# ALIZE-Speaker-Recognition/LIA_RAL

Measured on AMD Instinct MI355X. Metric: Gframe-Gaussian evals/s (UBM EM pass: LLK + full-posterior statistics), higher is better.
Workload: dtype f64; 1 GPU; TrainWorld EM: 2048-Gaussian diag UBM, 60-dim float32 frames, 10000000 frames per GPU resident in HBM, 1 EM iteration per step; gaussians=2048, dim=60, frames_per_gpu=10000000, partitioning=frames sharded per rank, one RCCL all-reduce of 247810 doubles per step

## Files before the change

lia_ral_amd/csrc/capi_gmm.hip:

```cpp
#include <math.h>
#include <stdarg.h>
#include <stdlib.h>

#include "ctx.h"
#include "gmm_kernels.h"
#include "tv_kernels.h"
#include "capi_gmm_util.h"

static thread_local char g_err[512] = "";

static thread_local gmmiv_kopts g_kopts_val;
static thread_local const gmmiv_kopts *g_kopts_src = nullptr;
const gmmiv_kopts &gmmiv_kopts_cur() { return g_kopts_val; }
void gmmiv_kopts_bind(const gmmiv_kopts *ko) { g_kopts_val = ko ? *ko : gmmiv_kopts(); g_kopts_src = ko; }

void gmmiv_set_error(const char *fmt, ...)
{
    va_list ap;
    va_start(ap, fmt);
    vsnprintf(g_err, sizeof(g_err), fmt, ap);
    va_end(ap);
}

bool gmmiv_is_device_ptr(const void *p)
// ... 55 lines not shown
        GCHK(krc);
    }
    return GMMIV_OK;
}

int run_lse(gmmiv_ctx *c, const gmmiv_gmm *g, const XView &xv, int dt, int64_t T, double **lse_out)
{
    void *lse;
    int rc = c->scratch(WS_LSE, (size_t)(T > 0 ? T : 1) * sizeof(double), &lse);
    if (rc) return rc;
    if (g->KS == GMMK_KS_GENERIC) {
        if ((rc = topc_big(c, g, xv, dt, T, 1, 1, -INFINITY, INFINITY, nullptr, nullptr, nullptr, nullptr, nullptr, (double *)lse))) return rc;
        GCHK(count_dead(c, (const double *)lse, T));
        *lse_out = (double *)lse;
        return GMMIV_OK;
    }
    c->t_begin("k_llk_mfma");
    GCHK(gmmk_llk(c->stream, g->KS, dt == GMMIV_F64, xv.d, T, xv.ldx, g->D, g->Pt, g->nct, (double *)lse, (int)(c->use_glds | (c->dbg << 8)), (int)c->wg_waves));
    c->t_end();
    GCHK(count_dead(c, (const double *)lse, T));
    *lse_out = (double *)lse;
    return GMMIV_OK;
}

static int64_t z_chunk_frames(gmmiv_ctx *c, const gmmiv_gmm *g)
{
    if (!c->stats_z || g->KS > 15 || c->wg_waves != 8) return 0;
    int64_t tc = gmmiv_z_budget_frames(c, g->nct, 16);
    const int64_t round = (int64_t)c->n_cu * 2 * 256;
    tc = tc >= round ? tc / round * round : tc / 64 * 64;
    return tc >= 4096 ? tc : 0;
}

static int llk_z_run(gmmiv_ctx *c, const gmmiv_gmm *g, const XView &xv, int dt, int64_t c0, int64_t n, double *lse, const gmmk_zview &z, bool first)
{
    c->t_begin("k_llk_mfma", first);
    GCHK(gmmk_llk_z(c->stream, g->KS, dt == GMMIV_F64, gmmiv_x_at(xv, dt, c0), n, xv.ldx, g->D, g->Pt, g->nct, lse,
                    (int)(c->use_glds | ((c->dbg & 15) << 8)), z));
    c->t_end();
    return GMMIV_OK;
}

int generic_gamma_gemm(gmmiv_ctx *c, const gmmiv_gmm *g, const XView &xv, int dt, int64_t t0, int64_t n, const double *lse, bool sq, int NC,
                       double *S)
{
    int rc;
    int64_t per = (int64_t)(((size_t)512 << 20) / ((size_t)g->C * sizeof(double)));
    if (per < 64) per = 64;
    per = per / 2 * 2;
    void *gam, *xa;
    const int64_t first = n < per ? n : per;
    if ((rc = c->scratch(WS_Z, (size_t)(first > 0 ? first : 1) * g->C * sizeof(double), &gam))) return rc;
    if ((rc = c->scratch(WS_INV, (size_t)(first > 0 ? first : 1) * NC * sizeof(double), &xa))) return rc;
    if (n <= 0) { GCHK(hipMemsetAsync(S, 0, (size_t)g->C * NC * sizeof(double), c->stream)); return GMMIV_OK; }
    for (int64_t b = 0; b < n; b += per) {
        const int64_t m = n - b < per ? n - b : per;
        c->t_begin("k_posteriors", b == 0);
        GCHK(gmmk_posteriors(c->stream, dt == GMMIV_F64, gmmiv_x_at(xv, dt, t0 + b), (long)m, xv.ldx, g->D, g->C, g->Cp64, g->meanT, g->ivT, g->lwc, lse + t0 + b,
                             (double *)gam));
        c->t_end();
        GCHK(gmmk_build_xa(c->stream, dt == GMMIV_F64, gmmiv_x_at(xv, dt, t0 + b), xv.ldx, g->D, (long)m, sq ? 1 : 0, NC, (double *)xa));
        GCHK(tvk_dgemm(c->stream, true, false, g->C, NC, (int)m, 1.0, (const double *)gam, g->C, 0, (const double *)xa, NC, 0, b == 0 ? 0.0 : 1.0, S, NC, 0, 1));
    }
    return GMMIV_OK;
}

extern "C" {

const char *gmmiv_last_error(void) { return g_err; }
const char *gmmiv_version(void) { return "gmmiv 0.1 (gfx950)"; }

int gmmiv_ctx_create(int device, void *stream, gmmiv_ctx **out)
{
    if (!out) { gmmiv_set_error("ctx_create: out == NULL"); return GMMIV_ERR_ARG; }
    int ndev = 0;
    hipError_t e = hipGetDeviceCount(&ndev);
    if (e != hipSuccess || ndev <= 0) {
        (void)hipGetLastError();
        gmmiv_set_error("ctx_create: no HIP device available (%s)", e == hipSuccess ? "count = 0" : hipGetErrorString(e));
        return GMMIV_ERR_HIP;
    }
    if (device < 0 || device >= ndev) { gmmiv_set_error("ctx_create: device %d out of range [0,%d)", device, ndev); return GMMIV_ERR_ARG; }
    GCHK(hipSetDevice(device));
    gmmiv_ctx *c = new gmmiv_ctx();
    c->device = device;
    if (stream == GMMIV_STREAM_DEFAULT || stream == (void *)hipStreamLegacy) { c->stream = nullptr; c->own_stream = false; }
    else if (stream) { c->stream = (hipStream_t)stream; c->own_stream = false; }
    else { GCHK(hipStreamCreateWithFlags(&c->stream, hipStreamNonBlocking)); c->own_stream = true; }
    hipDeviceProp_t prop;
    if (hipGetDeviceProperties(&prop, device) == hipSuccess) { c->n_cu = prop.multiProcessorCount; c->total_mem = prop.totalGlobalMem; }
    if (hipMalloc((void **)&c->d_zero_llk, 2 * sizeof(unsigned long long)) != hipSuccess || hipMemset(c->d_zero_llk, 0, 2 * sizeof(unsigned long long)) != hipSuccess) {
        (void)hipGetLastError();
        if (c->own_stream) (void)hipStreamDestroy(c->stream);
        delete c;
        gmmiv_set_error("ctx_create: hipMalloc of the context's device counters failed");
        return GMMIV_ERR_HIP;
    }
    c->d_screened = c->d_zero_llk + 1;
    *out = c;
    return GMMIV_OK;
}

void gmmiv_ctx_destroy(gmmiv_ctx *c)
{
    if (!c) return;
    (void)hipSetDevice(c->device);
    (void)hipStreamSynchronize(c->stream);
    for (gmmiv_comm *cm : std::vector<gmmiv_comm *>(c->comms)) gmmiv_comm_orphan(cm);
    for (int i = 0; i < WS_COUNT; ++i)
        if (c->ws[i]) (void)hipFree(c->ws[i]);
    for (int i = 0; i < gmmiv_ctx::NSLOT; ++i) {
        for (hipEvent_t e : c->ev0[i]) (void)hipEventDestroy(e);
        for (hipEvent_t e : c->ev1[i]) (void)hipEventDestroy(e);
    }
    if (c->d_zero_llk) (void)hipFree(c->d_zero_llk);
    if (c->own_stream) (void)hipStreamDestroy(c->stream);
    if (g_kopts_src == &c->ko) gmmiv_kopts_bind(nullptr);
    delete c;
}

int gmmiv_ctx_sync(gmmiv_ctx *c)
{
    if (!c) return GMMIV_ERR_ARG;
    GCHK(hipStreamSynchronize(c->stream));
    return GMMIV_OK;
}

void *gmmiv_ctx_stream(gmmiv_ctx *c) { return c ? (void *)c->stream : nullptr; }

long gmmiv_ctx_set_option(gmmiv_ctx *c, const char *key, long value)
{
    if (!c || !key) return -1;
    long *slot = nullptr;
    if (!strcmp(key, "glds")) slot = &c->use_glds;
    else if (!strcmp(key, "em_chunks")) slot = &c->em_chunks;
    else if (!strcmp(key, "timing")) slot = &c->timing;
    else if (!strcmp(key, "wg_waves")) slot = &c->wg_waves;
    else if (!strcmp(key, "dbg")) slot = &c->dbg;
    else if (!strcmp(key, "prune_log2")) slot = &c->prune_log2;
    else if (!strcmp(key, "stats_z")) slot = &c->stats_z;
    else if (!strcmp(key, "z_scratch_mb")) slot = &c->z_scratch_mb;
    else if (!strcmp(key, "models_scratch_mb")) slot = &c->models_scratch_mb;
    else if (!strcmp(key, "trials_scratch_mb")) slot = &c->trials_scratch_mb;
    else if (!strcmp(key, "trials_piece")) slot = &c->trials_piece;
    else if (!strcmp(key, "tv_batch")) slot = &c->tv_batch;
    else if (!strcmp(key, "tv_tett_direct")) slot = &c->tv_tett_direct;
    else if (!strcmp(key, "tv_stats_split")) slot = &c->tv_stats_split;
    else if (!strcmp(key, "topc_z")) slot = &c->topc_z;
// ... 598 lines not shown
    if (rc) return rc;
    GCHK(gmmk_fill_chunks(c->stream, (long *)buf, nseg, (long)per, (long)T));
    *dev = (long *)buf;
    return GMMIV_OK;
}

static int em_stats_z(gmmiv_ctx *c, const gmmiv_gmm *g, const XView &xv, int dt, int64_t T, int64_t Tc, double weight,
                      double *lse, int *nseg_out, void **part_out)
{
    int rc;
    const int ngrp = gmmk_stats_z_groups(g->nct);
    int nseg = c->em_chunks > 0 ? (int)c->em_chunks : (c->n_cu * gmmk_stats_z_wg_per_cu() + ngrp - 1) / ngrp;
    nseg = (nseg + 7) / 8 * 8;
    const int64_t first = T < Tc ? T : Tc;
    const int64_t cap = (first + 255) / 256;
    if (nseg > cap) nseg = (int)((cap + 7) / 8 * 8);
    const int64_t nchunk = (T + Tc - 1) / Tc;
    const int64_t lastn = T - (nchunk - 1) * Tc;
    void *seg, *part;
    if ((rc = c->scratch(WS_SEG, 2 * (size_t)(nseg + 1) * sizeof(long), &seg))) return rc;
    auto fill = [&](long *dst, int64_t n) {
        const int64_t per = ((n + nseg - 1) / nseg + 63) / 64 * 64;
        return gmmk_fill_chunks(c->stream, dst, nseg, (long)per, (long)n);
    };
    GCHK(fill((long *)seg, first));
    GCHK(fill((long *)seg + nseg + 1, lastn));
    gmmk_zview z;
    if ((rc = gmmiv_z_reserve(c, g->nct, first, !(c->dbg & 64), &z, nullptr))) return rc;
    const int RL = gmmk_rl_for_ks(g->KS);
    const size_t Cp = (size_t)g->nct * 16;
    if ((rc = c->scratch(WS_PART, (size_t)nseg * Cp * 2 * RL * sizeof(double), &part))) return rc;
    for (int64_t k = 0; k < nchunk; ++k) {
        const int64_t c0 = k * Tc, n = (k == nchunk - 1) ? lastn : Tc;
        if ((rc = llk_z_run(c, g, xv, dt, c0, n, lse + c0, z, k == 0))) return rc;
        GCHK(count_dead(c, lse + c0, n));
        c->t_begin("k_stats_z", k == 0);
        GCHK(gmmk_stats_z(c->stream, g->KS, 1, dt == GMMIV_F64, gmmiv_x_at(xv, dt, c0), xv.ldx, g->D, g->C, g->nct, z, weight,
                          (const long *)seg + (k == nchunk - 1 ? nseg + 1 : 0), nseg, (double *)part, nullptr, 0, k > 0, c->prune_thr()));
        c->t_end();
    }
    *nseg_out = nseg;
    *part_out = part;
    return GMMIV_OK;
}

int gmmiv_em_accumulate(gmmiv_ctx *c, const gmmiv_gmm *g, const void *x, int dt, int64_t T, int64_t ldx, double weight,
                        double *acc)
{
    int rc = check_model(c, g);
    if (rc) return rc;
    if (T < 0 || !acc || !(weight > 0.0)) { gmmiv_set_error("em_accumulate: bad argument (T >= 0, weight > 0, acc != NULL)"); return GMMIV_ERR_ARG; }
    const size_t nacc = gmmiv_em_acc_len(g->C, g->D);
    DevOut<double> o;
    if ((rc = o.init(c, WS_T0, acc, nacc, true))) return rc;
    if (T == 0) return o.finish();
    XView xv;
    if ((rc = xv.init(c, x, dt, T, ldx, g->D))) return rc;
    if ((rc = count_unusable(c, xv, dt, T, g->D))) return rc;
    const int64_t Tc = z_chunk_frames(c, g);
    if (Tc > 0) {
        void *lsew, *small, *part;
        int nseg = 0;
        if ((rc = c->scratch(WS_LSE, (size_t)T * sizeof(double), &lsew))) return rc;
        if ((rc = c->scratch(WS_SMALL, 3 * 256 * sizeof(double), &small))) return rc;
        if ((rc = em_stats_z(c, g, xv, dt, T, Tc, weight, (double *)lsew, &nseg, &part))) return rc;
        GCHK(gmmk_llk_finalize(c->stream, (const double *)lsew, T, -INFINITY, INFINITY, nullptr, (double *)small, 0.0, weight, nullptr,
                               o.d + nacc - 2, weight, o.d + nacc - 1));
        GCHK(gmmk_em_reduce(c->stream, (const double *)part, nseg, g->C, g->nct * 16, g->D, g->KS, o.d));
        return o.finish();
    }
    double *lse;
    if ((rc = run_lse(c, g, xv, dt, T, &lse))) return rc;
    void *small;
    if ((rc = c->scratch(WS_SMALL, 3 * 256 * sizeof(double), &small))) return rc;
    GCHK(gmmk_llk_finalize(c->stream, lse, T, -INFINITY, INFINITY, nullptr, (double *)small, 0.0, weight, nullptr,
                           o.d + nacc - 2, weight, o.d + nacc - 1));
    if (g->KS == GMMK_KS_GENERIC) {
        const int NC = 2 * g->D + 2;
        void *S;
        if ((rc = c->scratch(WS_PART, (size_t)g->C * NC * sizeof(double), &S))) return rc;
        if ((rc = generic_gamma_gemm(c, g, xv, dt, 0, T, lse, true, NC, (double *)S))) return rc;
        GCHK(gmmk_scatter_em(c->stream, g->C, g->D, NC, (const double *)S, weight, o.d));
        return o.finish();
    }
    const int nw = c->wg_waves == 8 ? 8 : 4;
    const int ngrp = (g->nct + nw - 1) / nw;
    int nseg = c->em_chunks > 0 ? (int)c->em_chunks : ((nw == 8 ? 2 : 4) * c->n_cu + ngrp - 1) / ngrp;
    nseg = (nseg + 7) / 8 * 8;
    const int64_t cap = (T + 4095) / 4096;
    if (nseg > cap) nseg = (int)cap;
    if (nseg < 1) nseg = 1;
    long *seg;
// ... 519 lines not shown
```

lia_ral_amd/csrc/ctx.h:

```cpp
#pragma once
#include <hip/hip_runtime.h>
#include <stdint.h>
#include <stdio.h>
#include <string.h>
#include <stdlib.h>
#include <time.h>

#include <map>
#include <string>
#include <vector>

#include "../../include/gmmiv.h"

void gmmiv_set_error(const char *fmt, ...);

#include "kopts.h"

#define GBIND(c)                                                                                    \
    do {                                                                                            \
        GCHK(hipSetDevice((c)->device));                                                            \
        gmmiv_kopts_bind(&(c)->ko);                                                                 \
    } while (0)

#define GCHK(expr)                                                                                  \
// ... 4 lines not shown
            return GMMIV_ERR_HIP;                                                                   \
        }                                                                                           \
    } while (0)

enum { WS_X = 0, WS_LSE, WS_PART, WS_SEG, WS_SMALL, WS_T0, WS_T1, WS_T2, WS_T3, WS_T4, WS_T5, WS_T6, WS_T7, WS_T8,
       WS_T9, WS_TIV, WS_LP, WS_AUX, WS_SLAB, WS_SLOTS, WS_FLAGS, WS_Z, WS_EIT, WS_INV,
       WS_GFLAG, WS_NORM, WS_FEAT_OFF, WS_FEAT_OUT, WS_FEAT_IDX, WS_FEAT_M0, WS_FEAT_M1, WS_FEAT_M2, WS_FEAT_M3,
       WS_NORM_OFF, WS_NORM_STATE, WS_NORM_DECAY,
       WS_MB_PT, WS_MB_TILES, WS_MB_IDS, WS_MB_SEG, WS_MB_OFF, WS_MB_FTILES, WS_MB_OFFSRC,
       WS_TR_IDX, WS_TR_NLLK, WS_TR_LLKW, WS_TR_TILES, WS_TR_TAB, WS_TR_PART, WS_TR_ROW,
       WS_COUNT };

struct gmmiv_ctx {
    int device = 0;
    hipStream_t stream = nullptr;
    bool own_stream = false;
    void *ws[WS_COUNT] = {};
    size_t ws_size[WS_COUNT] = {};
    long use_glds = 1;
    long em_chunks = 0;
    long timing = 0;
    long dbg = 0;
    long prune_log2 = 0;
    double prune_arg() const { return prune_log2 > 0 ? -(double)prune_log2 * 0.6931471805599453 : -__builtin_inf(); }
    double prune_thr() const { return prune_log2 > 0 ? __builtin_ldexp(1.0, -(int)prune_log2) : 0.0; }
    long wg_waves = 8;
    long stats_z = 1;
    long topc_use_lanes = 4;
    long topc_rank2 = 1;
    long topc_rank_direct = 0;
    long topc_fused = 1;
    long assume_finite = 0;
    unsigned long long *d_zero_llk = nullptr, *d_screened = nullptr;
    long topc_fallbacks = 0;
    long topc_z = 1;
    long tv_acc_mb = 8192;
    long tv_md_device = 1;
    long tv_mstep_solve = 1;
    long tv_stats_split = 1;
    long tv_tett_direct = 1;
    long tv_batch = 1024;
    gmmiv_kopts ko;
    struct Hook { gmmiv_hook_fn fn = nullptr; void *user = nullptr; void call() const { if (fn) fn(user); } };
    Hook hook_tv_a_ready, hook_md_factored;
    long z_scratch_mb = 16384;
    long models_scratch_mb = 2048;
    long trials_scratch_mb = 2048;
    long trials_piece = 0;
    int n_cu = 256;
    std::vector<double> plda_ftjf;
    struct PldaK { std::vector<double> K; double alpha; };
    std::map<long, PldaK> plda_k;
    std::vector<struct gmmiv_comm *> comms;
    size_t total_mem = 0;
    enum { NSLOT = 6 };
    std::vector<hipEvent_t> ev0[NSLOT], ev1[NSLOT];
    const char *ev_name[NSLOT] = {};
    int ev_used[NSLOT] = {};
    int ev_cur = -1, ev_last = -1;

    int scratch(int slot, size_t bytes, void **out)
    {
        if (bytes == 0) bytes = 8;
        if (ws_size[slot] < bytes) {
            if (ws[slot]) {
                GCHK(hipStreamSynchronize(stream));
// ... 133 lines not shown
```

lia_ral_amd/csrc/devutil.h:

```cpp
#pragma once
#include <hip/hip_runtime.h>
#include <stdint.h>

typedef double d4 __attribute__((ext_vector_type(4)));

#define MFMA_F64(a, b, c) __builtin_amdgcn_mfma_f64_16x16x4f64((a), (b), (c), 0, 0, 0)

#define GMMIV_NEG_BIG (-1.0e300)
#define GMMIV_ZERO_LLK (-745.1332191019412)
#define GMMIV_PAD_LOGIT (-1.0e9)

__device__ __forceinline__ double gexp(double x)
{
    x = fmax(x, -750.0);
    const double n = __builtin_rint(x * 1.4426950408889634074);
    double r = __builtin_fma(n, -6.93147180369123816490e-01, x);
    r = __builtin_fma(n, -1.90821492927058770002e-10, r);
    double p = 1.6059043836821613e-10;
    p = __builtin_fma(p, r, 2.08767569878681e-09);
    p = __builtin_fma(p, r, 2.505210838544172e-08);
    p = __builtin_fma(p, r, 2.755731922398589e-07);
    p = __builtin_fma(p, r, 2.7557319223985893e-06);
    p = __builtin_fma(p, r, 2.48015873015873e-05);
    p = __builtin_fma(p, r, 1.984126984126984e-04);
// ... 37 lines not shown
    double r = __builtin_fma(k, -0.021660849219188094, x);
    r = __builtin_fma(k, -1.733101967801894e-10, r);
    const int ki = (int)k;
    const double tj = tab[ki & 31];
    double p = 1.984126984126984e-04;
    p = __builtin_fma(p, r, 1.388888888888889e-03);
    p = __builtin_fma(p, r, 8.333333333333333e-03);
    p = __builtin_fma(p, r, 4.1666666666666664e-02);
    p = __builtin_fma(p, r, 1.6666666666666666e-01);
    p = __builtin_fma(p, r, 0.5);
    p = __builtin_fma(p, r, 1.0);
    p = p * r;
    int n = (ki >> 5) - E;
    n = n < -2000 ? -2000 : n;
    return __builtin_ldexp(__builtin_fma(tj, p, tj), n);
}
#ifndef GEXP_TAB_BITS
#define GEXP_TAB_BITS 11
#endif
#define GEXP_TAB_N (1 << GEXP_TAB_BITS)
#if GEXP_TAB_BITS == 11
#define GEXP_TAB_SCALE 2954.639443740597
#define GEXP_TAB_HI 0.00033845076904981397
#define GEXP_TAB_LO 2.7079718246904592e-12
#define GEXP_TAB_LN2N 0.00033845077175778578
#elif GEXP_TAB_BITS == 6
#define GEXP_TAB_SCALE 92.33248261689366
#define GEXP_TAB_HI 0.010830424609594047
#define GEXP_TAB_LO 8.66550983900947e-11
#define GEXP_TAB_LN2N 0.010830424696249145
#else
#error "GEXP_TAB_BITS must be 6 or 11"
#endif
__device__ __forceinline__ void gexp_tab_init(double *tab, int tid, int nthreads)
{
    for (int j = tid; j < GEXP_TAB_N; j += nthreads) tab[j] = exp2((double)j * (1.0 / GEXP_TAB_N));
}
__device__ __forceinline__ double gexp_tab_poly(double r)
{
#if GEXP_TAB_BITS == 11
    double p = 1.6666666666666666e-01;
#else
    double p = 8.333333333333333e-03;
    p = __builtin_fma(p, r, 4.1666666666666664e-02);
    p = __builtin_fma(p, r, 1.6666666666666666e-01);
#endif
    p = __builtin_fma(p, r, 0.5);
    p = __builtin_fma(p, r, 1.0);
    return p * r;
}
__device__ __forceinline__ void gexp_tab_reduce(double x, int &ki, double &r)
{
    const double k = __builtin_rint(x * GEXP_TAB_SCALE);
#ifdef GEXP_TAB_TWO_STEP
    r = __builtin_fma(k, -GEXP_TAB_HI, x);
    r = __builtin_fma(k, -GEXP_TAB_LO, r);
#else
    r = __builtin_fma(k, -GEXP_TAB_LN2N, x);
#endif
    ki = (int)k;
}
__device__ __forceinline__ double gexp_tab_finish(int ki, double r, int E, const double *tab)
{
    const double tj = tab[ki & (GEXP_TAB_N - 1)];
    return __builtin_ldexp(__builtin_fma(tj, gexp_tab_poly(r), tj), (ki >> GEXP_TAB_BITS) - E);
}
__device__ __forceinline__ double gexp_tab_scaled(double x, int E, const double *tab)
{
    int ki;
// ... 154 lines not shown
```

lia_ral_amd/csrc/gmm_kernels.h:

```cpp
#pragma once
#include <hip/hip_runtime.h>

#include "kopts.h"
#include "../../include/gmmiv.h"

#define GMMK_KS_GENERIC 99
#define GMMK_MAX_DIM 4096
int gmmk_ks_for_dim(int D);
int gmmk_rl_for_ks(int KS);
int gmmk_pack_model(hipStream_t st, int C, int D, int KS, int nct, int Cp64, const double *w, const double *mean,
                    const double *iv, double *a, double *lwc, double *Pt, double *meanT, double *ivT);
int gmmk_llk(hipStream_t st, int KS, int x_f64, const void *x, long T, long ldx, int D, const double *Pt, int nct,
             double *lse, int use_glds, int wg_waves);
int gmmk_llk_finalize(hipStream_t st, const double *lse, long T, double lo, double hi, double *llk_out,
                      double *partial , double scale_c, double scale_r, double *dst_clamped,
                      double *dst_raw, double scale_n = 0.0, double *dst_count = nullptr);
int gmmk_add_scalar(hipStream_t st, double *dst, double v);
int gmmk_count_dead(hipStream_t st, const double *lse, long T, unsigned long long *cnt);
int gmmk_rows_sum_groups(hipStream_t st, long n, int ngroups, const int *rb, const double *src, double *dst);
int gmmk_stats(hipStream_t st, int KS, int sq, int x_f64, const void *x, long ldx, int D, int C, const double *Pt,
               int nct, const double *lse, double lse_shift, const long *seg_begin, int nseg, double *out0,
               double *out1, int mode, int wg_waves, double prune_arg);
int gmmk_em_reduce(hipStream_t st, const double *part, int nseg, int C, int Cp, int D, int KS, double *acc);
int gmmk_em_get(hipStream_t st, int C, int D, const double *acc, const double *prev_mean, const double *prev_cov,
// ... 10 lines not shown
int gmmk_topc_determine_big(hipStream_t st, int x_f64, const void *x, long T, long ldx, int D, int C, int Cp,
                            const double *meanT, const double *ivT, const double *lwc, const double *w, int ctop,
                            int complete, double lo, double hi, int *idx, double *lk, double *nlk, double *nllk,
                            double *nw, double *llk, double *zs);
int gmmk_topc_use_big(hipStream_t st, int x_f64, const void *x, long T, long ldx, int D, const double *mean,
                      const double *iv, const double *lwc, int C, int ctop, const int *idx, const double *nllk, int complete,
                      double lo, double hi, double *llk);
int gmmk_topc_use(hipStream_t st, int x_f64, const void *x, long T, long ldx, int D, const double *mean,
                  const double *iv, const double *lwc, int C, int ctop, const int *idx, const double *nllk, int complete,
                  double lo, double hi, double *llk);
int gmmk_frame_moments(hipStream_t st, int x_f64, const void *x, long T, long ldx, int D, double *partial,
                       int max_blocks, double *acc);
int gmmk_variance_control(hipStream_t st, int C, int D, double *cov, double flooring, double ceiling,
                          const double *cov_signal, unsigned long long *counts);
int gmmk_reciprocal(hipStream_t st, long n, const double *in, double *out);
int gmmk_gather_frames(hipStream_t st, int x_f64, const void *x, long ldx, int D, const long *idx, long n, void *out);
int gmmk_segment_means(hipStream_t st, const double *v, long ld, const long *item, long nitem, double *part, const long *pair_off,
                       const long *pair_len, long npair, double *out);
int gmmk_topgauss_select(hipStream_t st, long T, int cap, double mass, int fixed_count, const double *w, int *idx, const double *lk,
                         const double *llk, int *count, double *snsw, double *snsl, unsigned long long *capped);
int gmmk_flag_frames(hipStream_t st, int x_f64, const void *x, long T, long ldx, int D, unsigned char *flag, int *any);
int gmmk_fill_chunks(hipStream_t st, long *dst, int nseg, long per, long n);
int gmmk_count_flags(hipStream_t st, const unsigned char *flag, long T, unsigned long long *cnt);
int gmmk_gather_runs(hipStream_t st, int x_f64, const void *x, long ldx, int D, const long *runs, long nrun, void *out);

struct gmmk_zview {
    double *zbuf;
    long nfb;
    int *eit;
    double *inv;
    int *efin;
};
int gmmk_llk_z(hipStream_t st, int KS, int x_f64, const void *x, long T, long ldx, int D, const double *Pt, int nct,
               double *lse, int use_glds, const gmmk_zview &z);
int gmmk_llk_models(hipStream_t st, int KS, int x_f64, const void *x, long ldx, int D, const double *Pt, long pt_stride, int nct,
                    const gmmiv_model_tile *tiles, long ntiles, double *lse, int use_glds);
int gmmk_llk_z_models(hipStream_t st, int KS, int x_f64, const void *x, long ldx, int D, const double *Pt, long pt_stride, int nct,
                      const gmmiv_model_tile *tiles, long ntiles, double *lse, int use_glds, const gmmk_zview &z);
int gmmk_const_models(hipStream_t st, int G, int C, int Cp, int D, const double *w, long sw, const double *mean, long sm, const double *iv,
                      long si, double *a, double *lwc);
int gmmk_pack_models(hipStream_t st, int n, const int *ids, int C, int Cp, int D, int KS, int nct, const double *mean, long sm,
                     const double *iv, long si, const double *a, double *Pt);
int gmmk_llk_seg_finalize(hipStream_t st, const double *lse, const long *sb, long nseg, double lo, double hi, double *llk_out, double *seg_sum,
                          double *seg_llk);
int gmmk_map_adapt_models(hipStream_t st, int G, int C, int D, const double *N, const double *F, const double *count, long count_stride,
                          const double *w0, const double *mean0, const double *cur, long cur_stride, int method, int mean_adapt,
                          int weight_adapt, double mean_reg, double weight_reg, double mean_alpha, double *mean_out, double *w_out);
int gmmk_map_adapt_models_full(hipStream_t st, int G, int C, int D, const double *N, const double *F, const double *S, const double *count,
                               long count_stride, const double *w0, const double *mean0, const double *cov0, const double *cur_mean,
                               long cur_mean_stride, const double *cur_cov, long cur_cov_stride, int method, int mean_adapt, int var_adapt,
                               int weight_adapt, double mean_reg, double var_reg, double weight_reg, double mean_alpha, double *mean_out,
                               double *cov_out, double *w_out, int *status);
int gmmk_normalize_models(hipStream_t st, int G, int C, int D, const double *w, long w_stride, double *mean, double *cov, int nb_it,
                          int mean_only);
int gmmk_acc_to_rows(hipStream_t st, int C, int D, const double *acc, double *Nrow, double *Frow, double *Srow);
int gmmk_topc_cap(void);
int gmmk_llk_topc(hipStream_t st, int KS, int x_f64, const void *x, long T, long ldx, int D, const double *Pt, int nct, int use_glds,
                  int ctop, double *cand, int *cnt, double *theta, double *slow, int *efin);
int gmmk_topc_rank(hipStream_t st, int x_f64, const void *x, long n, long ldx, int D, int C, const double *cand, const int *cnt,
                   const double *theta, const double *slow, const int *efin, const double *mean, const double *iv, const double *lwc,
                   const double *w, int ctop, int complete, double lo, double hi, int *idx, double *lk, double *nlk, double *nllk,
                   double *nw, double *llk, int *flag, long *redo, int stats, long *wide);
int gmmk_topc_scatter(hipStream_t st, long n, int ctop, const long *redo, const int *sidx, const double *slk, const double *snlk,
                      const double *snllk, const double *snw, const double *sllk, int *idx, double *lk, double *nlk, double *nllk, double *nw,
                      double *llk);
int gmmk_posteriors(hipStream_t st, int x_f64, const void *x, long T, long ldx, int D, int C, int Cp, const double *meanT,
                    const double *ivT, const double *lwc, const double *lse, double *gamma);
// ... 40 lines not shown
```

lia_ral_amd/csrc/gmm_kernels.hip:

```cpp
#include <atomic>
#include "devutil.h"
#include "lds_attr.h"
#include "gmm_kernels.h"

typedef double d2v __attribute__((ext_vector_type(2)));

__device__ __forceinline__ void gmm_const_one(int c, int C, int D, const double *__restrict__ w, const double *__restrict__ mean,
                                              const double *__restrict__ iv, double *__restrict__ a, double *__restrict__ logwcst)
{
    if (c >= C) { a[c] = GMMIV_NEG_BIG; logwcst[c] = GMMIV_NEG_BIG; return; }
    double sl = 0.0, sm = 0.0;
    for (int d = 0; d < D; ++d) {
        double v = iv[(size_t)c * D + d], m = mean[(size_t)c * D + d];
        sl += log(v);
        sm += m * m * v;
    }
    double lw = (w[c] > 0.0) ? log(w[c]) : GMMIV_NEG_BIG;
    double lc = lw - 0.5 * D * 1.8378770664093454836 + 0.5 * sl;
    lc = fmax(lc, GMMIV_NEG_BIG);
    logwcst[c] = lc;
    a[c] = fmax(lc - 0.5 * sm, GMMIV_NEG_BIG);
}
__global__ void k_gmm_const(int C, int Cp, int D, const double *__restrict__ w,
                            const double *__restrict__ mean, const double *__restrict__ iv,
// ... 44 lines not shown
    long total = (long)nct * (2 * KS + 2) * 64;
    if (e >= total) return;
    Pt[e] = gmm_pack_one(e, C, D, KS, mean, iv, a);
}
__global__ void k_gmm_pack_batch(int C, int Cp, int D, int KS, int nct, const int *__restrict__ ids, const double *__restrict__ mean, long sm,
                                 const double *__restrict__ iv, long si, const double *__restrict__ a, double *__restrict__ Pt)
{
    long e = (long)blockIdx.x * blockDim.x + threadIdx.x;
    long total = (long)nct * (2 * KS + 2) * 64;
    if (e >= total) return;
    const size_t g = (size_t)ids[blockIdx.y];
    Pt[(size_t)blockIdx.y * total + e] = gmm_pack_one(e, C, D, KS, mean + g * sm, iv + g * si, a + g * Cp);
}

__global__ void k_gmm_transpose(int C, int Cp, int D, const double *__restrict__ mean,
                                const double *__restrict__ iv, double *__restrict__ meanT,
                                double *__restrict__ ivT)
{
    long e = (long)blockIdx.x * blockDim.x + threadIdx.x;
    if (e >= (long)D * Cp) return;
    int c = e % Cp, d = e / Cp;
    meanT[e] = c < C ? mean[(size_t)c * D + d] : 0.0;
    ivT[e] = c < C ? iv[(size_t)c * D + d] : 0.0;
}

#define TOPC_CAP 256
#define GMMIV_MIN_FRAME_EXP (-1076)
#ifndef K1_ABL
#define K1_ABL 0
#endif
#ifndef K1_PLAIN_SHARED
#define K1_PLAIN_SHARED 1
#endif
template <int KS, typename XT, int NW, int MODE, bool MM = false>
__global__ __launch_bounds__(NW * 64, 2) void k_llk_mfma(const void *__restrict__ x, long T, long ldx, int D,
                                                  const double *__restrict__ Pt, int nct,
                                                  double *__restrict__ lse_out, int use_glds, int dbg,
                                                  double *__restrict__ zbuf, long nfb, int *__restrict__ eit,
                                                  double *__restrict__ inv_out, int *__restrict__ efin_out,
                                                  const gmmiv_model_tile *__restrict__ tiles, long pt_stride)
{
    constexpr bool WZ = MODE == 1, TC = MODE == 2;
    static_assert(!MM || (MODE != 2 && NW == 8), "a model per segment: plain and stored-likelihood modes, 8 waves");
    constexpr int NR = 2 * KS + 2;
    constexpr int GT = 2;
    constexpr int TILE_D = GT * NR * 64;
    constexpr int PIECES = TILE_D * 8 / 1024;
    extern __shared__ __attribute__((aligned(16))) char smem[];
    double *buf0 = (double *)smem;
    double *buf1 = buf0 + TILE_D;
    double *etab = buf1 + TILE_D;
    int *ccnt = (int *)(etab + GEXP_TAB_N);

    const int tid = threadIdx.x, lane = tid & 63, wave = tid >> 6;
    const int i16 = lane & 15, q = lane >> 4;
    long tb0 = (long)blockIdx.x * (NW * 32);
    long wlo = 0, whi = 0, olo = 0, ohi = 0;
    if constexpr (MM) {
        const gmmiv_model_tile me = tiles[blockIdx.x];
        tb0 = me.first; wlo = me.lo; whi = me.hi; olo = me.lo - me.pad_lo; ohi = me.hi + me.pad_hi;
        Pt += (size_t)me.model * pt_stride;
    }
    const long tb = tb0 + wave * 32;
    gexp_tab_init(etab, tid, NW * 64);
    if (TC) ccnt[tid >> 1] = 0;

    constexpr int NA = TC ? KS : 2 * KS;
    double A[2][NA];
#pragma unroll
    for (int h = 0; h < 2; ++h) {
        const long t = tb + h * 16 + i16;
#pragma unroll
        for (int s = 0; s < KS; ++s) {
            const int k = 4 * s + q;
            double v = 0.0;
            if ((MM ? (t >= wlo && t < whi) : t < T) && k < D) v = feat_load<XT>::get(x, t * ldx + k);
            A[h][s] = v;
            if (!TC) A[h][NA - KS + s] = v * v;
        }
    }

    const int ntiles = nct / GT;
    auto stage = [&](double *dst, int tile) {
        const char *src = (const char *)(Pt + (size_t)tile * TILE_D);
        if (use_glds) {
            if (PIECES % NW == 0) {
#pragma unroll
                for (int j = 0; j < PIECES / NW; ++j) {
                    const int p = wave + NW * j;
                    __builtin_amdgcn_global_load_lds(
                        (const __attribute__((address_space(1))) void *)(src + p * 1024 + lane * 16),
                        (__attribute__((address_space(3))) void *)((char *)dst + p * 1024), 16, 0, 0);
                }
            } else {
                for (int p = wave; p < PIECES; p += NW)
                    __builtin_amdgcn_global_load_lds(
                        (const __attribute__((address_space(1))) void *)(src + p * 1024 + lane * 16),
                        (__attribute__((address_space(3))) void *)((char *)dst + p * 1024), 16, 0, 0);
            }
        } else {
            for (int p = wave; p < PIECES; p += NW) {
                uint4 v = *(const uint4 *)(src + p * 1024 + lane * 16);
                *(uint4 *)((char *)dst + p * 1024 + lane * 16) = v;
            }
        }
    };

    double sacc[2][4];
    int E[2][4], nref[2][4];
#pragma unroll
    for (int h = 0; h < 2; ++h)
#pragma unroll
// ... 263 lines not shown
                    if (need & (1u << (h * 4 + r)))
                        sacc[h][r] += gexp_tab_scaled(acc[0][h][r], E[h][r], etab) + gexp_tab_scaled(acc[1][h][r], E[h][r], etab);
        }
    };
    stage(buf0, 0);
    __syncthreads();
    auto step = [&](int tl, bool staged, bool is_late, bool first) __attribute__((always_inline)) {
        double *cur = (tl & 1) ? buf1 : buf0;
        double *nxt = (tl & 1) ? buf0 : buf1;
        if (staged && (TC || dbg < 2) && !(K1_ABL & 16)) stage(nxt, tl + 1);
        if (!is_late) {
            mfma_phase(cur);
            epi_phase(tl);
        } else {
            if (!first) epi_phase(tl - 1);
            mfma_phase(cur);
        }
        if (WZ) {
            if (is_late) asm volatile("s_waitcnt vmcnt(0)" ::: "memory");
            if (!(K1_ABL & 16)) asm volatile("s_waitcnt lgkmcnt(0)\n\ts_barrier" ::: "memory");
        } else {
            __syncthreads();
        }
    };
    if (!late) {
        for (int tl = 0; tl + 1 < ntiles; ++tl) step(tl, true, false, false);
        if (ntiles > 0) step(ntiles - 1, false, false, false);
    } else {
        if (ntiles > 1) step(0, true, true, true);
        for (int tl = 1; tl + 1 < ntiles; ++tl) step(tl, true, true, false);
        if (ntiles > 0) step(ntiles - 1, false, true, ntiles == 1);
    }
    if (late && ntiles > 0) epi_phase(ntiles - 1);
#pragma unroll
    for (int h = 0; h < 2; ++h)
#pragma unroll
        for (int r = 0; r < 4; ++r) {
            int Em = E[h][r];
#pragma unroll
            for (int o = 1; o < 16; o <<= 1) { const int oe = __shfl_xor(Em, o, 64); Em = oe > Em ? oe : Em; }
            int sh = E[h][r] - Em;
            sh = sh < -2000 ? -2000 : sh;
            double sv = __builtin_ldexp(sacc[h][r], sh);
#pragma unroll
            for (int o = 1; o < 16; o <<= 1) sv += shfl_xor_f64(sv, o);
            const long t = tb + h * 16 + q + 4 * r;
            if (TC) {
                if (i16 == 0 && t < T) { lse_out[t] = (double)thf[h][r]; inv_out[t] = sv; efin_out[t] = Em; }
                continue;
            }
            if (i16 == 0 && (MM ? (t >= wlo && t < whi) : t < T)) {
                const bool ok = sv > 0.0 && sv < __builtin_inf() && Em > GMMIV_MIN_FRAME_EXP;
                lse_out[t] = ok ? log(sv) + (double)Em * 0.693147180559945309417 : -__builtin_inf();
                if (WZ) { inv_out[t] = ok ? 1.0 / sv : 0.0; efin_out[t] = ok ? Em : 0; }
            }
        }
    if (TC) {
        __syncthreads();
        const long t = (long)blockIdx.x * (NW * 32) + tid;
        if (tid < NW * 32 && t < T) eit[t] = ccnt[tid];
    }
}

__global__ __launch_bounds__(256) void k_llk_finalize(const double *__restrict__ lse, long T, double lo,
                                                     double hi, double *__restrict__ llk_out,
                                                     double *__restrict__ partial)
{
    __shared__ double red[3][4];
    double sc = 0.0, sr = 0.0, sn = 0.0;
    for (long t = (long)blockIdx.x * blockDim.x + threadIdx.x; t < T; t += (long)gridDim.x * blockDim.x) {
        const double v = lse[t];
        const double c = fmin(fmax(v, lo), hi);
        if (llk_out) llk_out[t] = c;
        sc += c;
        const bool fin = v > -__builtin_inf() && v < __builtin_inf();
        sr += fin ? v : 0.0;
        sn += fin ? 1.0 : 0.0;
    }
    sc = wave_sum_f64(sc);
    sr = wave_sum_f64(sr);
    sn = wave_sum_f64(sn);
    const int lane = threadIdx.x & 63, wave = threadIdx.x >> 6;
    if (lane == 0) { red[0][wave] = sc; red[1][wave] = sr; red[2][wave] = sn; }
    __syncthreads();
    if (threadIdx.x == 0) {
        partial[3 * blockIdx.x] = red[0][0] + red[0][1] + red[0][2] + red[0][3];
        partial[3 * blockIdx.x + 1] = red[1][0] + red[1][1] + red[1][2] + red[1][3];
        partial[3 * blockIdx.x + 2] = red[2][0] + red[2][1] + red[2][2] + red[2][3];
    }
// ... 602 lines not shown
        for (int l = 0; l < 64; ++l) t += red[slot][l];
        acc[e] += t;
    }
}

#define HIPCHK(e)                                                         \
    do {                                                                  \
        hipError_t _e = (e);                                              \
        if (_e != hipSuccess) return (int)_e;                             \
    } while (0)

int gmmk_ks_for_dim(int D)
{
    if (D <= 16) return 4;
    if (D <= 32) return 8;
    if (D <= 60) return 15;
    if (D <= 80) return 20;
    return D <= GMMK_MAX_DIM ? GMMK_KS_GENERIC : 0;
}
int gmmk_rl_for_ks(int KS) { return ((4 * KS + 2 + 31) / 32) * 32; }

int gmmk_pack_model(hipStream_t st, int C, int D, int KS, int nct, int Cp64, const double *w, const double *mean,
                    const double *iv, double *a, double *lwc, double *Pt, double *meanT, double *ivT)
{
    const int Cp = Cp64 > nct * 16 ? Cp64 : nct * 16;
    k_gmm_const<<<(Cp + 255) / 256, 256, 0, st>>>(C, Cp, D, w, mean, iv, a, lwc);
    long total = (long)nct * (2 * KS + 2) * 64;
    if (KS != GMMK_KS_GENERIC) k_gmm_pack<<<(unsigned)((total + 255) / 256), 256, 0, st>>>(C, D, KS, nct, mean, iv, a, Pt);
    long tt = (long)D * Cp64;
    k_gmm_transpose<<<(unsigned)((tt + 255) / 256), 256, 0, st>>>(C, Cp64, D, mean, iv, meanT, ivT);
    return (int)hipGetLastError();
}

template <int KS, typename XT, int NW, int MODE>
static int launch_llk(hipStream_t st, const void *x, long T, long ldx, int D, const double *Pt, int nct,
                      double *lse, int use_glds, const gmmk_zview &z = gmmk_zview{})
{
    constexpr int NR = 2 * KS + 2;
    const size_t lds = 2 * 2 * NR * 64 * sizeof(double) + GEXP_TAB_N * sizeof(double) + (MODE == 2 ? NW * 32 * sizeof(int) : 0);
    HIPCHK((gmmiv_lds_attr<k_llk_mfma<KS, XT, NW, MODE>>(lds)));
    const unsigned grid = (unsigned)((T + NW * 32 - 1) / (NW * 32));
    k_llk_mfma<KS, XT, NW, MODE><<<grid, NW * 64, lds, st>>>(x, T, ldx, D, Pt, nct, lse, use_glds & 1, use_glds >> 8, z.zbuf, z.nfb, z.eit, z.inv, z.efin, nullptr, 0);
    return (int)hipGetLastError();
}

template <int KS, typename XT, int MODE>
static int launch_llk_models(hipStream_t st, const void *x, long ldx, int D, const double *Pt, long pt_stride, int nct, const gmmiv_model_tile *tiles,
                             long ntiles, double *lse, int use_glds, const gmmk_zview &z)
{
    constexpr int NR = 2 * KS + 2;
    const size_t lds = 2 * 2 * NR * 64 * sizeof(double) + GEXP_TAB_N * sizeof(double);
    HIPCHK((gmmiv_lds_attr<k_llk_mfma<KS, XT, 8, MODE, true>>(lds)));
    k_llk_mfma<KS, XT, 8, MODE, true><<<(unsigned)ntiles, 8 * 64, lds, st>>>(x, 0, ldx, D, Pt, nct, lse, use_glds & 1, 0, z.zbuf, z.nfb, z.eit, z.inv, z.efin, tiles, pt_stride);
    return (int)hipGetLastError();
}
#define MM_CASE(K, MODE)                                                                                                  \
    case K:                                                                                                               \
        return x_f64 ? launch_llk_models<K, double, MODE>(st, x, ldx, D, Pt, pt_stride, nct, tiles, ntiles, lse, use_glds, z) \
                     : launch_llk_models<K, float, MODE>(st, x, ldx, D, Pt, pt_stride, nct, tiles, ntiles, lse, use_glds, z);
int gmmk_llk_models(hipStream_t st, int KS, int x_f64, const void *x, long ldx, int D, const double *Pt, long pt_stride, int nct,
                    const gmmiv_model_tile *tiles, long ntiles, double *lse, int use_glds)
{
    if (ntiles <= 0) return 0;
    const gmmk_zview z = {};
    switch (KS) {
        MM_CASE(4, 0) MM_CASE(8, 0) MM_CASE(15, 0)
    }
    return -1;
}
int gmmk_llk_z_models(hipStream_t st, int KS, int x_f64, const void *x, long ldx, int D, const double *Pt, long pt_stride, int nct,
                      const gmmiv_model_tile *tiles, long ntiles, double *lse, int use_glds, const gmmk_zview &z)
{
    if (ntiles <= 0) return 0;
    switch (KS) {
        MM_CASE(4, 1) MM_CASE(8, 1) MM_CASE(15, 1)
    }
    return -1;
}
#undef MM_CASE

int gmmk_const_models(hipStream_t st, int G, int C, int Cp, int D, const double *w, long sw, const double *mean, long sm, const double *iv,
                      long si, double *a, double *lwc)
{
    if (G <= 0) return 0;
    k_gmm_const_batch<<<dim3((unsigned)((Cp + 255) / 256), (unsigned)G), 256, 0, st>>>(C, Cp, D, w, sw, mean, sm, iv, si, a, lwc);
    return (int)hipGetLastError();
// ... 230 lines not shown
{
    if (G <= 0 || nb_it <= 0) return 0;
    const long n = (long)G * D;
    k_normalize_models<<<(unsigned)((n + 63) / 64), 64, 0, st>>>(G, C, D, w, w_stride, mean, cov, nb_it, mean_only);
    return (int)hipGetLastError();
}
int gmmk_acc_to_rows(hipStream_t st, int C, int D, const double *acc, double *Nrow, double *Frow, double *Srow)
{
    const long n = (long)C * (1 + 2 * D);
    k_acc_to_rows<<<(unsigned)((n + 255) / 256), 256, 0, st>>>(C, D, acc, Nrow, Frow, Srow);
    return (int)hipGetLastError();
}

int gmmk_llk(hipStream_t st, int KS, int x_f64, const void *x, long T, long ldx, int D, const double *Pt, int nct,
             double *lse, int use_glds, int wg_waves)
{
    if (T <= 0) return 0;
    if (T <= 32768 && gmmiv_kopts_cur().short_calls) wg_waves = 4;
#define CASE(K)                                                                                      \
    case K:                                                                                          \
        if (wg_waves == 8)                                                                           \
            return x_f64 ? launch_llk<K, double, 8, 0>(st, x, T, ldx, D, Pt, nct, lse, use_glds) \
                         : launch_llk<K, float, 8, 0>(st, x, T, ldx, D, Pt, nct, lse, use_glds); \
        return x_f64 ? launch_llk<K, double, 4, 0>(st, x, T, ldx, D, Pt, nct, lse, use_glds)     \
                     : launch_llk<K, float, 4, 0>(st, x, T, ldx, D, Pt, nct, lse, use_glds);
    switch (KS) {
        CASE(4) CASE(8) CASE(15) CASE(20)
    }
#undef CASE
    return -1;
}

int gmmk_llk_z(hipStream_t st, int KS, int x_f64, const void *x, long T, long ldx, int D, const double *Pt, int nct,
               double *lse, int use_glds, const gmmk_zview &z)
{
    if (T <= 0) return 0;
    const bool small = T <= 32768 && gmmiv_kopts_cur().short_calls;
#define CASE(K)                                                                                   \
    case K:                                                                                       \
        if (small)                                                                                \
            return x_f64 ? launch_llk<K, double, 4, 1>(st, x, T, ldx, D, Pt, nct, lse, use_glds, z) \
                         : launch_llk<K, float, 4, 1>(st, x, T, ldx, D, Pt, nct, lse, use_glds, z); \
        return x_f64 ? launch_llk<K, double, 8, 1>(st, x, T, ldx, D, Pt, nct, lse, use_glds, z)   \
                     : launch_llk<K, float, 8, 1>(st, x, T, ldx, D, Pt, nct, lse, use_glds, z);
    switch (KS) {
        CASE(4) CASE(8) CASE(15)
    }
#undef CASE
    return -1;
}

int gmmk_topc_cap(void) { return TOPC_CAP; }
int gmmk_llk_topc(hipStream_t st, int KS, int x_f64, const void *x, long T, long ldx, int D, const double *Pt, int nct, int use_glds,
                  int ctop, double *cand, int *cnt, double *theta, double *slow, int *efin)
{
    if (T <= 0) return 0;
    if (ctop < 1 || ctop > 16) return -1;
    use_glds = (use_glds & 1) | (ctop << 8);
    const bool small = T <= 32768 && gmmiv_kopts_cur().short_calls;
    const gmmk_zview tc = {cand, 0, cnt, slow, efin};
#define CASE(K)                                                                                                                    \
    case K:                                                                                                                        \
        if (small)                                                                                                                 \
            return x_f64 ? launch_llk<K, double, 4, 2>(st, x, T, ldx, D, Pt, nct, theta, use_glds, tc)        \
                         : launch_llk<K, float, 4, 2>(st, x, T, ldx, D, Pt, nct, theta, use_glds, tc);        \
        return x_f64 ? launch_llk<K, double, 8, 2>(st, x, T, ldx, D, Pt, nct, theta, use_glds, tc)            \
                     : launch_llk<K, float, 8, 2>(st, x, T, ldx, D, Pt, nct, theta, use_glds, tc);
    switch (KS) {
        CASE(4) CASE(8) CASE(15)
    }
// ... 467 lines not shown
```

lia_ral_amd/csrc/kopts.h:

```cpp
#pragma once

struct gmmiv_kopts {
    int z_waves = 8;
    int z_tv4 = 1;
    int z_depth_em = 2, z_depth_tv = 4;
    int gemm_remap = 1;
    int gemm_clamp = 1;
    int gemm_narrow = 1;
    int short_calls = 1;
    int gemm_nt80 = 1;
    int chol_lds = 1;
    int chol_gemm = 0;
    int chol_waves = 8;
    int chol_flow = 1;
};
const gmmiv_kopts &gmmiv_kopts_cur();
void gmmiv_kopts_bind(const gmmiv_kopts *ko);
```

Baseline: 128.4 Gframe-Gaussian/s.

## Fold dead/unusable frame counting into LLK kernel and preload exp table

The log-likelihood kernel in the chunked EM path now counts non-finite frame likelihoods and sanitized (unusable) input features itself, using wave ballots and one atomic per wave. This removes the separate count_dead pass per chunk and the count_unusable pass over all frames. The per-block exp2 table is no longer computed in each block; it is built once per context and copied into LDS with global_load_lds. The trade-offs are extra ballots and atomics in the kernel and a new dependency on a context-owned device table.

```diff
diff --git a/lia_ral_amd/csrc/capi_gmm.hip b/lia_ral_amd/csrc/capi_gmm.hip
--- a/lia_ral_amd/csrc/capi_gmm.hip
+++ b/lia_ral_amd/csrc/capi_gmm.hip
@@ -111,11 +111,13 @@
     return tc >= 4096 ? tc : 0;
 }
 
-static int llk_z_run(gmmiv_ctx *c, const gmmiv_gmm *g, const XView &xv, int dt, int64_t c0, int64_t n, double *lse, const gmmk_zview &z, bool first)
+static int llk_z_run(gmmiv_ctx *c, const gmmiv_gmm *g, const XView &xv, int dt, int64_t c0, int64_t n, double *lse, const gmmk_zview &z, bool first,
+                     bool count_in_kernel = false)
 {
     c->t_begin("k_llk_mfma", first);
     GCHK(gmmk_llk_z(c->stream, g->KS, dt == GMMIV_F64, gmmiv_x_at(xv, dt, c0), n, xv.ldx, g->D, g->Pt, g->nct, lse,
-                    (int)(c->use_glds | ((c->dbg & 15) << 8)), z));
+                    (int)(c->use_glds | ((c->dbg & 15) << 8)), z, count_in_kernel ? c->d_zero_llk : nullptr,
+                    count_in_kernel && !c->assume_finite ? c->d_screened : nullptr));
     c->t_end();
     return GMMIV_OK;
 }
@@ -176,6 +178,16 @@
         return GMMIV_ERR_HIP;
     }
     c->d_screened = c->d_zero_llk + 1;
+    if (hipMalloc((void **)&c->d_exp_tab, gmmk_exp_tab_doubles() * sizeof(double)) != hipSuccess || gmmk_exp_tab_fill(c->stream, c->d_exp_tab) != 0) {
+        (void)hipGetLastError();
+        if (c->d_exp_tab) (void)hipFree(c->d_exp_tab);
+        (void)hipFree(c->d_zero_llk);
+        if (c->own_stream) (void)hipStreamDestroy(c->stream);
+        delete c;
+        gmmiv_set_error("ctx_create: the exp table of the log-likelihood kernel could not be set up");
+        return GMMIV_ERR_HIP;
+    }
+    c->ko.exp_tab = c->d_exp_tab;
     *out = c;
     return GMMIV_OK;
 }
@@ -193,6 +205,7 @@
         for (hipEvent_t e : c->ev1[i]) (void)hipEventDestroy(e);
     }
     if (c->d_zero_llk) (void)hipFree(c->d_zero_llk);
+    if (c->d_exp_tab) (void)hipFree(c->d_exp_tab);
     if (c->own_stream) (void)hipStreamDestroy(c->stream);
     if (g_kopts_src == &c->ko) gmmiv_kopts_bind(nullptr);
     delete c;
@@ -857,8 +870,7 @@
     if ((rc = c->scratch(WS_PART, (size_t)nseg * Cp * 2 * RL * sizeof(double), &part))) return rc;
     for (int64_t k = 0; k < nchunk; ++k) {
         const int64_t c0 = k * Tc, n = (k == nchunk - 1) ? lastn : Tc;
-        if ((rc = llk_z_run(c, g, xv, dt, c0, n, lse + c0, z, k == 0))) return rc;
-        GCHK(count_dead(c, lse + c0, n));
+        if ((rc = llk_z_run(c, g, xv, dt, c0, n, lse + c0, z, k == 0, true))) return rc;
         c->t_begin("k_stats_z", k == 0);
         GCHK(gmmk_stats_z(c->stream, g->KS, 1, dt == GMMIV_F64, gmmiv_x_at(xv, dt, c0), xv.ldx, g->D, g->C, g->nct, z, weight,
                           (const long *)seg + (k == nchunk - 1 ? nseg + 1 : 0), nseg, (double *)part, nullptr, 0, k > 0, c->prune_thr()));
@@ -881,8 +893,8 @@
     if (T == 0) return o.finish();
     XView xv;
     if ((rc = xv.init(c, x, dt, T, ldx, g->D))) return rc;
-    if ((rc = count_unusable(c, xv, dt, T, g->D))) return rc;
     const int64_t Tc = z_chunk_frames(c, g);
+    if (Tc <= 0 && (rc = count_unusable(c, xv, dt, T, g->D))) return rc;
     if (Tc > 0) {
         void *lsew, *small, *part;
         int nseg = 0;
diff --git a/lia_ral_amd/csrc/ctx.h b/lia_ral_amd/csrc/ctx.h
--- a/lia_ral_amd/csrc/ctx.h
+++ b/lia_ral_amd/csrc/ctx.h
@@ -60,6 +60,7 @@
     long topc_fused = 1;
     long assume_finite = 0;
     unsigned long long *d_zero_llk = nullptr, *d_screened = nullptr;
+    double *d_exp_tab = nullptr;
     long topc_fallbacks = 0;
     long topc_z = 1;
     long tv_acc_mb = 8192;
diff --git a/lia_ral_amd/csrc/devutil.h b/lia_ral_amd/csrc/devutil.h
--- a/lia_ral_amd/csrc/devutil.h
+++ b/lia_ral_amd/csrc/devutil.h
@@ -93,9 +93,10 @@
 #else
 #error "GEXP_TAB_BITS must be 6 or 11"
 #endif
+__device__ __forceinline__ double gexp_tab_entry(int j) { return exp2((double)j * (1.0 / GEXP_TAB_N)); }
 __device__ __forceinline__ void gexp_tab_init(double *tab, int tid, int nthreads)
 {
-    for (int j = tid; j < GEXP_TAB_N; j += nthreads) tab[j] = exp2((double)j * (1.0 / GEXP_TAB_N));
+    for (int j = tid; j < GEXP_TAB_N; j += nthreads) tab[j] = gexp_tab_entry(j);
 }
 __device__ __forceinline__ double gexp_tab_poly(double r)
 {
diff --git a/lia_ral_amd/csrc/gmm_kernels.h b/lia_ral_amd/csrc/gmm_kernels.h
--- a/lia_ral_amd/csrc/gmm_kernels.h
+++ b/lia_ral_amd/csrc/gmm_kernels.h
@@ -66,7 +66,9 @@
     int *efin;
 };
 int gmmk_llk_z(hipStream_t st, int KS, int x_f64, const void *x, long T, long ldx, int D, const double *Pt, int nct,
-               double *lse, int use_glds, const gmmk_zview &z);
+               double *lse, int use_glds, const gmmk_zview &z, unsigned long long *cnt_dead = nullptr, unsigned long long *cnt_screened = nullptr);
+size_t gmmk_exp_tab_doubles(void);
+int gmmk_exp_tab_fill(hipStream_t st, double *tab);
 int gmmk_llk_models(hipStream_t st, int KS, int x_f64, const void *x, long ldx, int D, const double *Pt, long pt_stride, int nct,
                     const gmmiv_model_tile *tiles, long ntiles, double *lse, int use_glds);
 int gmmk_llk_z_models(hipStream_t st, int KS, int x_f64, const void *x, long ldx, int D, const double *Pt, long pt_stride, int nct,
diff --git a/lia_ral_amd/csrc/gmm_kernels.hip b/lia_ral_amd/csrc/gmm_kernels.hip
--- a/lia_ral_amd/csrc/gmm_kernels.hip
+++ b/lia_ral_amd/csrc/gmm_kernels.hip
@@ -100,16 +100,19 @@
 #ifndef K1_PLAIN_SHARED
 #define K1_PLAIN_SHARED 1
 #endif
-template <int KS, typename XT, int NW, int MODE, bool MM = false>
+template <int KS, typename XT, int NW, int MODE, bool MM = false, bool CNT = false>
 __global__ __launch_bounds__(NW * 64, 2) void k_llk_mfma(const void *__restrict__ x, long T, long ldx, int D,
                                                   const double *__restrict__ Pt, int nct,
                                                   double *__restrict__ lse_out, int use_glds, int dbg,
                                                   double *__restrict__ zbuf, long nfb, int *__restrict__ eit,
                                                   double *__restrict__ inv_out, int *__restrict__ efin_out,
-                                                  const gmmiv_model_tile *__restrict__ tiles, long pt_stride)
+                                                  const gmmiv_model_tile *__restrict__ tiles, long pt_stride,
+                                                  const double *__restrict__ exp_tab, unsigned long long *__restrict__ cnt_dead,
+                                                  unsigned long long *__restrict__ cnt_screened)
 {
     constexpr bool WZ = MODE == 1, TC = MODE == 2;
     static_assert(!MM || (MODE != 2 && NW == 8), "a model per segment: plain and stored-likelihood modes, 8 waves");
+    static_assert(!CNT || (MODE == 1 && !MM), "counting the degenerate frames: stored-likelihood mode, one model");
     constexpr int NR = 2 * KS + 2;
     constexpr int GT = 2;
     constexpr int TILE_D = GT * NR * 64;
@@ -130,11 +133,24 @@
         Pt += (size_t)me.model * pt_stride;
     }
     const long tb = tb0 + wave * 32;
-    gexp_tab_init(etab, tid, NW * 64);
+    {
+        constexpr int TAB_PIECES = GEXP_TAB_N * 8 / 1024;
+        if (use_glds && TAB_PIECES > 0 && TAB_PIECES % NW == 0) {
+#pragma unroll
+            for (int j = 0; j < TAB_PIECES / NW; ++j) {
+                const int p = wave + NW * j;
+                __builtin_amdgcn_global_load_lds((const __attribute__((address_space(1))) void *)((const char *)exp_tab + p * 1024 + lane * 16),
+                                                 (__attribute__((address_space(3))) void *)((char *)etab + p * 1024), 16, 0, 0);
+            }
+        } else {
+            for (int j = tid; j < GEXP_TAB_N; j += NW * 64) etab[j] = exp_tab[j];
+        }
+    }
     if (TC) ccnt[tid >> 1] = 0;
 
     constexpr int NA = TC ? KS : 2 * KS;
     double A[2][NA];
+    bool subst[2] = {false, false};
 #pragma unroll
     for (int h = 0; h < 2; ++h) {
         const long t = tb + h * 16 + i16;
@@ -142,10 +158,25 @@
         for (int s = 0; s < KS; ++s) {
             const int k = 4 * s + q;
             double v = 0.0;
-            if ((MM ? (t >= wlo && t < whi) : t < T) && k < D) v = feat_load<XT>::get(x, t * ldx + k);
+            if ((MM ? (t >= wlo && t < whi) : t < T) && k < D) {
+                if constexpr (CNT) {
+                    const XT raw = ((const XT *)x)[t * ldx + k], sane = feat_sane(raw);
+                    subst[h] |= sane != raw;
+                    v = (double)sane;
+                } else {
+                    v = feat_load<XT>::get(x, t * ldx + k);
+                }
+            }
             A[h][s] = v;
             if (!TC) A[h][NA - KS + s] = v * v;
         }
+    }
+    if constexpr (CNT) {
+        unsigned long long b0 = __builtin_amdgcn_ballot_w64(subst[0]), b1 = __builtin_amdgcn_ballot_w64(subst[1]);
+        b0 |= b0 >> 32; b0 |= b0 >> 16;
+        b1 |= b1 >> 32; b1 |= b1 >> 16;
+        const int ns = __builtin_popcount((unsigned)(b0 & 0xffff)) + __builtin_popcount((unsigned)(b1 & 0xffff));
+        if (cnt_screened && ns != 0 && lane == 0) atomicAdd(cnt_screened, (unsigned long long)ns);
     }
 
     const int ntiles = nct / GT;
@@ -475,6 +506,7 @@
         if (ntiles > 0) step(ntiles - 1, false, true, ntiles == 1);
     }
     if (late && ntiles > 0) epi_phase(ntiles - 1);
+    int ndead = 0;
 #pragma unroll
     for (int h = 0; h < 2; ++h)
 #pragma unroll
@@ -492,12 +524,19 @@
                 if (i16 == 0 && t < T) { lse_out[t] = (double)thf[h][r]; inv_out[t] = sv; efin_out[t] = Em; }
                 continue;
             }
+            bool dead = false;
             if (i16 == 0 && (MM ? (t >= wlo && t < whi) : t < T)) {
                 const bool ok = sv > 0.0 && sv < __builtin_inf() && Em > GMMIV_MIN_FRAME_EXP;
-                lse_out[t] = ok ? log(sv) + (double)Em * 0.693147180559945309417 : -__builtin_inf();
+                const double lv = ok ? log(sv) + (double)Em * 0.693147180559945309417 : -__builtin_inf();
+                lse_out[t] = lv;
                 if (WZ) { inv_out[t] = ok ? 1.0 / sv : 0.0; efin_out[t] = ok ? Em : 0; }
-            }
-        }
+                if (CNT) dead = !(lv > -__builtin_inf() && lv < __builtin_inf());
+            }
+            if constexpr (CNT) ndead += __builtin_popcountll(__builtin_amdgcn_ballot_w64(dead));
+        }
+    if constexpr (CNT) {
+        if (ndead != 0 && lane == 0) atomicAdd(cnt_dead, (unsigned long long)ndead);
+    }
     if (TC) {
         __syncthreads();
         const long t = (long)blockIdx.x * (NW * 32) + tid;
@@ -1166,15 +1205,31 @@
     return (int)hipGetLastError();
 }
 
-template <int KS, typename XT, int NW, int MODE>
+__global__ __launch_bounds__(256) void k_gexp_tab_fill(double *__restrict__ tab)
+{
+    const int j = blockIdx.x * blockDim.x + threadIdx.x;
+    if (j < GEXP_TAB_N) tab[j] = gexp_tab_entry(j);
+}
+size_t gmmk_exp_tab_doubles(void) { return GEXP_TAB_N; }
+int gmmk_exp_tab_fill(hipStream_t st, double *tab)
+{
+    k_gexp_tab_fill<<<(GEXP_TAB_N + 255) / 256, 256, 0, st>>>(tab);
+    return (int)hipGetLastError();
+}
+static const double *llk_exp_tab() { return gmmiv_kopts_cur().exp_tab; }
+
+template <int KS, typename XT, int NW, int MODE, bool CNT = false>
 static int launch_llk(hipStream_t st, const void *x, long T, long ldx, int D, const double *Pt, int nct,
-                      double *lse, int use_glds, const gmmk_zview &z = gmmk_zview{})
+                      double *lse, int use_glds, const gmmk_zview &z = gmmk_zview{}, unsigned long long *cnt_dead = nullptr,
+                      unsigned long long *cnt_screened = nullptr)
 {
     constexpr int NR = 2 * KS + 2;
+    const double *tab = llk_exp_tab();
+    if (!tab) return (int)hipErrorInvalidValue;
     const size_t lds = 2 * 2 * NR * 64 * sizeof(double) + GEXP_TAB_N * sizeof(double) + (MODE == 2 ? NW * 32 * sizeof(int) : 0);
-    HIPCHK((gmmiv_lds_attr<k_llk_mfma<KS, XT, NW, MODE>>(lds)));
+    HIPCHK((gmmiv_lds_attr<k_llk_mfma<KS, XT, NW, MODE, false, CNT>>(lds)));
     const unsigned grid = (unsigned)((T + NW * 32 - 1) / (NW * 32));
-    k_llk_mfma<KS, XT, NW, MODE><<<grid, NW * 64, lds, st>>>(x, T, ldx, D, Pt, nct, lse, use_glds & 1, use_glds >> 8, z.zbuf, z.nfb, z.eit, z.inv, z.efin, nullptr, 0);
+    k_llk_mfma<KS, XT, NW, MODE, false, CNT><<<grid, NW * 64, lds, st>>>(x, T, ldx, D, Pt, nct, lse, use_glds & 1, use_glds >> 8, z.zbuf, z.nfb, z.eit, z.inv, z.efin, nullptr, 0, tab, cnt_dead, cnt_screened);
     return (int)hipGetLastError();
 }
 
@@ -1184,8 +1239,10 @@
 {
     constexpr int NR = 2 * KS + 2;
     const size_t lds = 2 * 2 * NR * 64 * sizeof(double) + GEXP_TAB_N * sizeof(double);
+    const double *tab = llk_exp_tab();
+    if (!tab) return (int)hipErrorInvalidValue;
     HIPCHK((gmmiv_lds_attr<k_llk_mfma<KS, XT, 8, MODE, true>>(lds)));
-    k_llk_mfma<KS, XT, 8, MODE, true><<<(unsigned)ntiles, 8 * 64, lds, st>>>(x, 0, ldx, D, Pt, nct, lse, use_glds & 1, 0, z.zbuf, z.nfb, z.eit, z.inv, z.efin, tiles, pt_stride);
+    k_llk_mfma<KS, XT, 8, MODE, true><<<(unsigned)ntiles, 8 * 64, lds, st>>>(x, 0, ldx, D, Pt, nct, lse, use_glds & 1, 0, z.zbuf, z.nfb, z.eit, z.inv, z.efin, tiles, pt_stride, tab, nullptr, nullptr);
     return (int)hipGetLastError();
 }
 #define MM_CASE(K, MODE)                                                                                                  \
@@ -1482,10 +1539,24 @@
 }
 
 int gmmk_llk_z(hipStream_t st, int KS, int x_f64, const void *x, long T, long ldx, int D, const double *Pt, int nct,
-               double *lse, int use_glds, const gmmk_zview &z)
+               double *lse, int use_glds, const gmmk_zview &z, unsigned long long *cnt_dead, unsigned long long *cnt_screened)
 {
     if (T <= 0) return 0;
     const bool small = T <= 32768 && gmmiv_kopts_cur().short_calls;
+    if (cnt_dead) {
+#define CASE(K)                                                                                              \
+    case K:                                                                                                  \
+        if (small)                                                                                           \
+            return x_f64 ? launch_llk<K, double, 4, 1, true>(st, x, T, ldx, D, Pt, nct, lse, use_glds, z, cnt_dead, cnt_screened) \
+                         : launch_llk<K, float, 4, 1, true>(st, x, T, ldx, D, Pt, nct, lse, use_glds, z, cnt_dead, cnt_screened); \
+        return x_f64 ? launch_llk<K, double, 8, 1, true>(st, x, T, ldx, D, Pt, nct, lse, use_glds, z, cnt_dead, cnt_screened)   \
+                     : launch_llk<K, float, 8, 1, true>(st, x, T, ldx, D, Pt, nct, lse, use_glds, z, cnt_dead, cnt_screened);
+        switch (KS) {
+            CASE(4) CASE(8) CASE(15)
+        }
+#undef CASE
+        return -1;
+    }
 #define CASE(K)                                                                                   \
     case K:                                                                                       \
         if (small)                                                                                \
diff --git a/lia_ral_amd/csrc/kopts.h b/lia_ral_amd/csrc/kopts.h
--- a/lia_ral_amd/csrc/kopts.h
+++ b/lia_ral_amd/csrc/kopts.h
@@ -13,6 +13,7 @@
     int chol_gemm = 0;
     int chol_waves = 8;
     int chol_flow = 1;
+    const double *exp_tab = nullptr;
 };
 const gmmiv_kopts &gmmiv_kopts_cur();
 void gmmiv_kopts_bind(const gmmiv_kopts *ko);
```

Measured after the change: 128.9 Gframe-Gaussian/s (median of 6 runs). About the same (+0.3%).
